# danping/CoSLAM

Hardware: AMD Instinct MI355X
Metric: frames/sec for track+local-BA loop, 8 cams 640x480 x 2000 feats (one frame = all 8 cameras) (higher is better)
Workload: dtype f32 (KLT, f16 pyramid storage) + f64 (pose, BA)

## Files before the change

coslam_amd/csrc/klt_detect.hip:

```cpp
#include "klt_front_dev.h"

#pragma clang fp contract(off)


namespace {

__device__ __forceinline__ void suppress_at(float* corner, int W, int H, float s, float t) {
    if (!(s >= 0.0f && t >= 0.0f)) return;
    float fx = floorf(s * (float)W), fy = floorf(t * (float)H);
    if (fx >= (float)W || fy >= (float)H) return;
    corner[(size_t)(int)fy * W + (int)fx] = -1e30f;
}

__global__ void k_suppress_list(float* corner, int W, int H, int n, const float* __restrict__ list3) {
    int k = blockIdx.x * blockDim.x + threadIdx.x;
    if (k < n) suppress_at(corner, W, H, list3[3 * k], list3[3 * k + 1]);
}

__global__ void k_post_track(const float* __restrict__ feat, int N, cs_klt_feature* __restrict__ dest, int* ctr,
                             float* corner, int W, int H, int doSuppress) {
    int i = blockIdx.x * blockDim.x + threadIdx.x;
    if (i >= N) return;
    float X = feat[3 * i], Y = feat[3 * i + 1], gain = feat[3 * i + 2];
    if (X >= 0) {
        dest[i].status = 0;
        dest[i].pos[0] = X;
        dest[i].pos[1] = Y;
        dest[i].gain = gain;
        dest[i].fed = -1;
        if (doSuppress) suppress_at(corner, W, H, X, Y);
    } else {
        dest[i].status = -1;
        dest[i].fed = -1;
    }
}

__global__ void k_clear_dest(cs_klt_feature* dest, int N) {
    int i = blockIdx.x * blockDim.x + threadIdx.x;
    if (i < N) {
        dest[i].status = -1;
        dest[i].fed = -1;
    }
}

constexpr int NTW = 64, NTH = 16;

__device__ __forceinline__ unsigned part1by1(unsigned v) {
    v &= 0xffffu;
    v = (v | (v << 8)) & 0x00ff00ffu;
    v = (v | (v << 4)) & 0x0f0f0f0fu;
    v = (v | (v << 2)) & 0x33333333u;
    v = (v | (v << 1)) & 0x55555555u;
    return v;
}

struct CsNonmaxArgs {
    const float* in;
    int W, H, d;
    float* out;
    CsCand* cand;
    int maxCand;
    int* ctr;
};

__device__ __forceinline__ void nonmax_body(const CsNonmaxArgs& Z, int bx, int by, int tid, float* smem) {
    const float* __restrict__ in = Z.in;
    float* __restrict__ out = Z.out;
    CsCand* __restrict__ cand = Z.cand;
    int* ctr = Z.ctr;
    const int W = Z.W, H = Z.H, d = Z.d, maxCand = Z.maxCand;
    const int RW = NTW + 2 * d, RH = NTH + 2 * d;
    float* raw = smem;
    float* rowres = smem + RH * RW;
    const int x0 = bx * NTW, y0 = by * NTH;
    for (int base = tid; base < RH * RW; base += 8 * 256) {
        float tv[8];
#pragma unroll
        for (int u = 0; u < 8; ++u) {
            const int i = base + 256 * u;
            const int ly = i / RW, lx = i - ly * RW;
            const int gx = cs_clampi(x0 + lx - d, 0, W - 1), gy = cs_clampi(y0 + ly - d, 0, H - 1);
            tv[u] = in[(size_t)gy * W + gx];
        }
#pragma unroll
        for (int u = 0; u < 8; ++u) {
            const int i = base + 256 * u;
            if (i < RH * RW) raw[i] = tv[u];
        }
    }
    __syncthreads();
    for (int i = tid; i < RH * NTW; i += 256) {
        int ly = i / NTW, lx = i - ly * NTW;
        const float* r = raw + ly * RW + lx + d;
        float m = r[0];
        for (int k = -d; k < 0; ++k) {
            float cn = fabsf(r[k]);
            m = (cn >= fabsf(m)) ? (-cn) : m;
        }
        for (int k = 1; k <= d; ++k) {
            float cn = fabsf(r[k]);
            m = (cn >= fabsf(m)) ? (-cn) : m;
        }
        rowres[i] = m;
    }
    __syncthreads();
    const int lx = tid & (NTW - 1), x = x0 + lx;
    for (int ly = tid / NTW; ly < NTH; ly += 256 / NTW) {
        int y = y0 + ly;
        if (x >= W || y >= H) continue;
        const float* r = rowres + (ly + d) * NTW + lx;
        float m = r[0];
        for (int k = -d; k < 0; ++k) {
            float cn = fabsf(r[k * NTW]);
            m = (cn >= fabsf(m)) ? (-cn) : m;
        }
        for (int k = 1; k <= d; ++k) {
            float cn = fabsf(r[k * NTW]);
            m = (cn >= fabsf(m)) ? (-cn) : m;
        }
        out[(size_t)y * W + x] = m;
        if (m > 0.0f) {
            int slot = atomicAdd(&ctr[0], 1);
            if (slot < maxCand) {
                CsCand cd;
                cd.key = part1by1((unsigned)x) | (part1by1((unsigned)y) << 1);
                cd.x = ((float)x + 0.5f) / (float)W;
                cd.y = ((float)y + 0.5f) / (float)H;
                cd.c = m;
                cand[slot] = cd;
            }
        }
    }
}

struct CsNonmaxBatch {
    int W, H, d, maxCand;
    CsNonmaxCam cam[CS_MAX_CAMS];
};
__device__ __forceinline__ CsNonmaxArgs nonmax_args(const CsNonmaxBatch& B, int c) {
    CsNonmaxArgs Z = {B.cam[c].in, B.W, B.H, B.d, B.cam[c].out, B.cam[c].cand, B.maxCand, B.cam[c].ctr};
    return Z;
}

__global__ __launch_bounds__(256) void k_nonmax_compact(CsNonmaxBatch B) {
    extern __shared__ __attribute__((aligned(16))) float smem[];
    nonmax_body(nonmax_args(B, blockIdx.z), blockIdx.x, blockIdx.y, threadIdx.x, smem);
}

struct CsSelectArgs {
    const CsCand* cand;
    int maxCand, cap, maxKeepFixed;
    int* rankM;
    CsCand* sel;
};

__device__ __forceinline__ void select_fill_body(const CsSelectArgs& Q, const CsFillArgs& A) {
    __shared__ float cs[1024];
    __shared__ unsigned ks[1024];
    __shared__ int rs[1024];
    __shared__ int part[1024];
    const int tid = threadIdx.x;
    const int N = A.N;
    __shared__ int nTrackedSh;
    {
        int c = 0;
        if (A.mode == 2)
            for (int i = tid; i < N; i += 1024) c += (A.dest[i].status >= 0) ? 1 : 0;
        part[tid] = c;
        __syncthreads();
        for (int s = 512; s > 0; s >>= 1) {
            if (tid < s) part[tid] += part[tid + s];
            __syncthreads();
        }
        if (tid == 0) nTrackedSh = part[0];
        __syncthreads();
    }
    const int nTracked = nTrackedSh;
    const int n = min(A.ctr[0], Q.maxCand);
    const int nK = min(n, Q.cap);
    int maxKeep = (Q.maxKeepFixed >= 0) ? Q.maxKeepFixed : (N - nTracked);
    if (maxKeep < 0) maxKeep = 0;
    const int nSel = min(nK, maxKeep);
    for (int i0 = 0; i0 < n; i0 += 1024) {
        const int i = i0 + tid;
        const unsigned ki = (i < n) ? Q.cand[i].key : 0u;
        int r = 0;
        for (int base = 0; base < n; base += 1024) {
            const int j = base + tid;
            ks[tid] = (j < n) ? Q.cand[j].key : 0xffffffffu;
            __syncthreads();
            const int m = min(1024, n - base);
            for (int q = 0; q < m; ++q) r += (ks[q] < ki) ? 1 : 0;
            __syncthreads();
        }
        if (i < n) Q.rankM[i] = r;
    }
    __syncthreads();
    for (int i0 = 0; i0 < n; i0 += 1024) {
        const int i = i0 + tid;
        CsCand me;
        me.key = 0;
        me.x = me.y = me.c = 0;
        int myRank = 0x7fffffff;
        if (i < n) {
            me = Q.cand[i];
            myRank = Q.rankM[i];
        }
        if (nK <= maxKeep) {
            if (i < n && myRank < nK) Q.sel[myRank] = me;
            continue;
        }
        int r = 0;
        for (int base = 0; base < n; base += 1024) {
            const int j = base + tid;
            const bool ok = (j < n);
            cs[tid] = ok ? Q.cand[j].c : 0.0f;
            ks[tid] = ok ? Q.cand[j].key : 0u;
            rs[tid] = ok ? Q.rankM[j] : 0x7fffffff;
            __syncthreads();
            const int m = min(1024, n - base);
            for (int q = 0; q < m; ++q) {
                const bool in = rs[q] < nK;
                const bool before = (cs[q] > me.c) || (cs[q] == me.c && ks[q] < me.key);
                r += (in && before) ? 1 : 0;
            }
            __syncthreads();
        }
        if (i < n && myRank < nK && r < maxKeep) Q.sel[r] = me;
    }
    __syncthreads();
    const int chunk = (N + 1023) / 1024;
    const int lo = min(tid * chunk, N), hi = min(lo + chunk, N);
    int nDead = 0;
    for (int i = lo; i < hi; ++i) nDead += (A.mode == 2) ? (A.dest[i].status < 0 ? 1 : 0) : 1;
    part[tid] = nDead;
    __syncthreads();
    for (int s = 1; s < 1024; s <<= 1) {
        int v = (tid >= s) ? part[tid - s] : 0;
        __syncthreads();
        part[tid] += v;
        __syncthreads();
    }
    int r = part[tid] - nDead;
    for (int i = lo; i < hi; ++i) {
        bool dead = (A.mode == 2) ? (A.dest[i].status < 0) : true;
        float lx, ly, lz;
        if (dead) {
            if (r < nSel) {
                CsCand c = Q.sel[r];
                cs_klt_feature f;
                f.status = 1;
                f.pos[0] = c.x;
                f.pos[1] = c.y;
                f.gain = (A.mode == 2) ? c.c : (A.withGain ? 1.0f : c.c);
                f.fed = -1;
                A.dest[i] = f;
                lx = c.x;
                ly = c.y;
                lz = (A.mode == 2 || A.withGain) ? 1.0f : c.c;
            } else if (A.mode == 1 && r < nSel + A.nPresentGiven) {
                int q = r - nSel;
                cs_klt_feature f;
                f.status = 1;
                f.pos[0] = A.present3[3 * q];
                f.pos[1] = A.present3[3 * q + 1];
                f.gain = A.withGain ? 1.0f : 0.0f;
                f.fed = q;
                A.dest[i] = f;
                lx = f.pos[0];
                ly = f.pos[1];
                lz = f.gain;
            } else {
                A.dest[i].status = -1;
                if (A.mode != 1) A.dest[i].fed = -1;
                lx = ly = -1.0f;
                lz = (A.mode == 2 || A.withGain) ? 1.0f : -1.0f;
            }
            ++r;
        } else {
            lx = A.dest[i].pos[0];
            ly = A.dest[i].pos[1];
            lz = 1.0f;
        }
        A.list_a[3 * i] = lx;
        A.list_a[3 * i + 1] = ly;
        A.list_a[3 * i + 2] = lz;
        if (A.list_b) {
            A.list_b[3 * i] = lx;
            A.list_b[3 * i + 1] = ly;
            A.list_b[3 * i + 2] = lz;
        }
    }
    if (tid == 0) {
        int nPres = (A.mode == 2) ? nTracked : (A.mode == 1 ? min(A.nPresentGiven, max(N - nSel, 0)) : 0);
        A.ctr[1] = nTracked;
        A.ctr[2] = nSel;
        A.counts[0] = nSel + nPres;
        A.counts[1] = (A.mode == 2) ? nTracked : 0;
        A.counts[2] = A.ctr[0];
        A.counts[3] = nSel;
        A.ctr[0] = 0;
    }
    if (A.tagWord && tid == 0) *A.tagWord += 1u;
}

struct CsSelectBatch {
    int maxCand, cap;
    CsSelectCam cam[CS_MAX_CAMS];
};
__device__ __forceinline__ CsSelectArgs select_args(const CsSelectBatch& B, int c) {
    CsSelectArgs Q = {B.cam[c].cand, B.maxCand, B.cap, B.cam[c].maxKeepFixed, B.cam[c].rankM, B.cam[c].sel};
    return Q;
}

__global__ __launch_bounds__(1024) void k_select_fill(CsSelectBatch B) {
    select_fill_body(select_args(B, blockIdx.x), B.cam[blockIdx.x].fill);
}

struct CsLevel0Batch {
    int W, H;
    float minCornerness, lox, loy, hix, hiy;
    int nbx, nby;
    CsFrontCam cam[CS_MAX_CAMS];
};

__global__ __launch_bounds__(256) void k_tail_nonmax_level0(CsNonmaxBatch Z, int nax, int nA, CsLevel0Batch Y) {
    extern __shared__ __attribute__((aligned(16))) float smem[];
    const int b = blockIdx.x, c = blockIdx.y;
    if (b < nA) {
        nonmax_body(nonmax_args(Z, c), b % nax, b / nax, threadIdx.x, smem);
    } else {
        const int q = b - nA;
        const CsFrontCam& F = Y.cam[c];
        cs_level0_body<true>(F.img, Y.W, Y.H, F.pyr, F.corner, Y.minCornerness, Y.lox, Y.loy, Y.hix, Y.hiy, nullptr, q % Y.nbx,
                             q / Y.nbx, Y.nbx, Y.nby, threadIdx.x, *(CsLevel0Lds<true>*)smem);
    }
}

struct CsTailPyr {
    cs_texel* pyr[CS_MAX_CAMS];
};
__global__ __launch_bounds__(1024) void k_tail_select_down(CsSelectBatch B, CsTailPyr P, CsDownFused F, int ntx, int nty) {
    extern __shared__ __attribute__((aligned(16))) unsigned char down_smem[];
    const int c = blockIdx.y;
    if (blockIdx.x == 0) {
        select_fill_body(select_args(B, c), B.cam[c].fill);
        return;
    }
    if (threadIdx.x >= 256) return;
    const int t = blockIdx.x - 1;
    cs_down_body(P.pyr[c], F, t % ntx, t / ntx, threadIdx.x, (cs_texel*)down_smem, true);
}

__global__ __launch_bounds__(1024) void k_counts_track(const cs_klt_feature* __restrict__ dest, int N, int* counts, int* ctr,
                                                       unsigned* tagWord) {
    __shared__ int part[1024];
    const int tid = threadIdx.x;
    int c = 0;
    for (int i = tid; i < N; i += 1024) c += (dest[i].status >= 0) ? 1 : 0;
    part[tid] = c;
    __syncthreads();
    for (int s = 512; s > 0; s >>= 1) {
        if (tid < s) part[tid] += part[tid + s];
        __syncthreads();
    }
    if (tid == 0) {
        counts[0] = part[0];
        counts[1] = part[0];
        counts[2] = 0;
        counts[3] = 0;
        if (ctr) ctr[0] = 0;
    }
    if (tagWord && tid == 0) *tagWord += 1u;
}

}

int cs_launch_suppress_list(float* corner, int W, int H, int n, const float* d_list3, hipStream_t stream) {
    if (n <= 0) return CS_OK;
    hipLaunchKernelGGL(k_suppress_list, dim3((n + 255) / 256), dim3(256), 0, stream, corner, W, H, n, d_list3);
    CS_CHECK_LAUNCH();
    return CS_OK;
}

int cs_launch_post_track(const float* feat, int N, cs_klt_feature* dest, int* ctr, float* corner, int W, int H,
                         int doSuppress, hipStream_t stream) {
    hipLaunchKernelGGL(k_post_track, dim3((N + 255) / 256), dim3(256), 0, stream, feat, N, dest, ctr, corner, W, H,
                       doSuppress);
    CS_CHECK_LAUNCH();
    return CS_OK;
}

int cs_launch_clear_dest(cs_klt_feature* dest, int N, hipStream_t stream) {
    hipLaunchKernelGGL(k_clear_dest, dim3((N + 255) / 256), dim3(256), 0, stream, dest, N);
    CS_CHECK_LAUNCH();
    return CS_OK;
}

size_t cs_nonmax_lds_bytes(int d) { return sizeof(float) * ((size_t)(NTH + 2 * d) * (NTW + 2 * d) + (size_t)(NTH + 2 * d) * NTW); }

static int fill_nonmax_batch(CsNonmaxBatch& B, const CsNonmaxCam* cams, int n, int W, int H, int d, int maxCand) {
    if (n < 1 || n > CS_MAX_CAMS) {
        cs_set_error("detector: %d cameras (1..%d)", n, CS_MAX_CAMS);
        return CS_ERR_INVALID;
    }
    memset(&B, 0, sizeof(B));
    B.W = W;
    B.H = H;
    B.d = d;
    B.maxCand = maxCand;
    for (int c = 0; c < n; ++c) B.cam[c] = cams[c];
    return CS_OK;
}
static void fill_select_batch(CsSelectBatch& B, const CsSelectCam* cams, int n, int maxCand, int cap) {
    memset(&B, 0, sizeof(B));
    B.maxCand = maxCand;
    B.cap = cap;
    for (int c = 0; c < n; ++c) B.cam[c] = cams[c];
}

int cs_launch_nonmax_compact(const CsNonmaxCam* cams, int n, int W, int H, int d, int maxCand, hipStream_t stream) {
    size_t lds = cs_nonmax_lds_bytes(d);
    if (lds > 160 * 1024) {
        cs_set_error("minDistance %d needs %zu B of LDS (> 160 KiB)", d, lds);
        return CS_ERR_INVALID;
    }
    CsNonmaxBatch B;
    int rc = fill_nonmax_batch(B, cams, n, W, H, d, maxCand);
    if (rc) return rc;
    dim3 grid((W + NTW - 1) / NTW, (H + NTH - 1) / NTH, n);
    hipLaunchKernelGGL(k_nonmax_compact, grid, dim3(256), lds, stream, B);
    CS_CHECK_LAUNCH();
    return CS_OK;
}

int cs_nonmax_prepare(int d) {
    size_t lds = cs_nonmax_lds_bytes(d);
    if (lds > 64 * 1024) {
        hipError_t e = hipFuncSetAttribute((const void*)k_nonmax_compact, hipFuncAttributeMaxDynamicSharedMemorySize,
                                           (int)lds);
        if (e != hipSuccess) {
            cs_set_error("hipFuncSetAttribute(maxDynamicShared=%zu) failed: %s", lds, hipGetErrorString(e));
            return CS_ERR_HIP;
        }
    }
    return CS_OK;
}

int cs_launch_select_fill(const CsSelectCam* cams, int n, int maxCand, int cap, hipStream_t stream) {
    if (n < 1 || n > CS_MAX_CAMS) {
        cs_set_error("selection: %d cameras (1..%d)", n, CS_MAX_CAMS);
        return CS_ERR_INVALID;
    }
    CsSelectBatch B;
    fill_select_batch(B, cams, n, maxCand, cap);
    hipLaunchKernelGGL(k_select_fill, dim3(n), dim3(1024), 0, stream, B);
    CS_CHECK_LAUNCH();
    return CS_OK;
}

int cs_launch_counts_track(const cs_klt_feature* dest, int N, int* counts, int* ctr, unsigned* tagWord, hipStream_t stream) {
    hipLaunchKernelGGL(k_counts_track, dim3(1), dim3(1024), 0, stream, dest, N, counts, ctr, tagWord);
    CS_CHECK_LAUNCH();
    return CS_OK;
}

int cs_launch_tail_with_next_front(const CsNonmaxCam* nm, const CsSelectCam* sel, const CsFrontCam* next, int n, int W, int H,
                                   int d, int maxCand, int cap, const CsPyrLayout& lay, int tap_mode, float minCornerness,
                                   float margin, hipStream_t stream) {
    size_t ldsA = cs_nonmax_lds_bytes(d);
    if (ldsA < sizeof(CsLevel0Lds<true>)) ldsA = sizeof(CsLevel0Lds<true>);
    if (ldsA > 64 * 1024) {
        cs_set_error("fused detector tail: minDistance %d needs %zu B of LDS", d, ldsA);
        return CS_ERR_INVALID;
    }
    CsNonmaxBatch Z;
    int rc = fill_nonmax_batch(Z, nm, n, W, H, d, maxCand);
    if (rc) return rc;
    const int nax = (W + NTW - 1) / NTW, nay = (H + NTH - 1) / NTH;
    CsLevel0Batch Y;
    memset(&Y, 0, sizeof(Y));
    Y.W = W;
    Y.H = H;
    Y.minCornerness = minCornerness;
    Y.lox = margin / (float)W;
    Y.loy = margin / (float)H;
    Y.hix = 1.0f - margin / (float)W;
    Y.hiy = 1.0f - margin / (float)H;
    Y.nbx = (W + FTW - 1) / FTW;
    Y.nby = (H + FTH - 1) / FTH;
    CsTailPyr P;
    memset(&P, 0, sizeof(P));
    for (int c = 0; c < n; ++c) {
        Y.cam[c] = next[c];
        P.pyr[c] = next[c].pyr;
    }
    hipLaunchKernelGGL(k_tail_nonmax_level0, dim3(nax * nay + Y.nbx * Y.nby, n), dim3(256), ldsA, stream, Z, nax, nax * nay, Y);
    CsSelectBatch B;
    fill_select_batch(B, sel, n, maxCand, cap);
    if (lay.L >= 2) {
        CsDownFused F;
        int ntx, nty;
        size_t lds;
        rc = cs_down_fused_plan(lay, tap_mode, &F, &ntx, &nty, &lds);
        if (rc) return rc;
        hipLaunchKernelGGL(k_tail_select_down, dim3(1 + ntx * nty, n), dim3(1024), lds, stream, B, P, F, ntx, nty);
        rc = cs_launch_pyr_down_tail(P.pyr, n, lay, tap_mode, F.NL + 1, stream);
        if (rc) return rc;
    } else {
        hipLaunchKernelGGL(k_select_fill, dim3(n), dim3(1024), 0, stream, B);
    }
    CS_CHECK_LAUNCH();
    return CS_OK;
}
```

include/coslam_hip.h:

```cpp
#ifndef COSLAM_HIP_H
#define COSLAM_HIP_H

#include <stddef.h>
#include <stdint.h>

#ifdef __cplusplus
extern "C" {
#endif

#define CS_OK 0
#define CS_ERR_INVALID (-1)
#define CS_ERR_NO_DEVICE (-2)
#define CS_ERR_HIP (-3)
#define CS_ERR_ALLOC (-4)
#define CS_ERR_NUMERIC (-5)

int cs_version(void);
const char* cs_last_error(void);
int cs_debug_set(const char* key, int value);
int cs_device_count(void);


typedef struct cs_klt_feature {
    int status;
    float pos[2];
    float gain;
    int fed;
} cs_klt_feature;

typedef struct cs_klt_config {
    int nIterations, nLevels, levelSkip, windowWidth;
    float trackBorderMargin, convergenceThreshold, SSD_Threshold;
    int trackWithGain;
    int minDistance;
    float minCornerness, detectBorderMargin;
} cs_klt_config;

void cs_klt_config_default(cs_klt_config* cfg);

typedef struct cs_klt cs_klt;

cs_klt* cs_klt_create(const cs_klt_config* cfg, int device, int tap_mode);
void cs_klt_destroy(cs_klt* k);

int cs_klt_allocate(cs_klt* k, int width, int height, int nLevels, int featuresWidth, int featuresHeight,
                    int pointListWidth, int pointListHeight);
int cs_klt_deallocate(cs_klt* k);

int cs_klt_set_border_margin(cs_klt* k, float margin);
int cs_klt_set_convergence_threshold(cs_klt* k, float thr);
int cs_klt_set_ssd_threshold(cs_klt* k, float thr);

int cs_klt_detect(cs_klt* k, const uint8_t* image, int* nDetectedFeatures, cs_klt_feature* dest);
int cs_klt_detect_present(cs_klt* k, const uint8_t* image, int* nDetectedFeatures, cs_klt_feature* dest, int nPresent,
                          const float* present);
int cs_klt_redetect(cs_klt* k, const uint8_t* image, int* nNewFeatures, cs_klt_feature* dest);
int cs_klt_track(cs_klt* k, const uint8_t* image, int* nPresentFeatures, cs_klt_feature* dest);
int cs_klt_redetect_async_h(cs_klt* k, const unsigned char* image);
int cs_klt_fetch(cs_klt* k, int* nNew, cs_klt_feature* dest);
int cs_klt_feed(cs_klt* k, int npts, const float* featPts, int* trackIds, int* nFed);
int cs_klt_feed_dev(cs_klt* k, int npts, const float* d_featPts, int* d_trackIds, int* d_nFed);
int cs_klt_advance(cs_klt* k);

int cs_klt_set_stream(cs_klt* k, void* hip_stream);
int cs_klt_detect_dev(cs_klt* k, const void* d_image, void* d_dest, void* d_counts);
int cs_klt_redetect_dev(cs_klt* k, const void* d_image, void* d_dest, void* d_counts);
int cs_klt_track_dev(cs_klt* k, const void* d_image, void* d_dest, void* d_counts);
int cs_klt_prefetch_dev(cs_klt* k, const void* d_image_next);
int cs_klt_synchronize(cs_klt* k);
int cs_klt_enable_graphs(cs_klt* k, int on);
int cs_klt_set_fused(cs_klt* k, int on);
int cs_klt_set_cu_count(cs_klt* k, int n_cus);
int cs_klt_set_xcd_placement(cs_klt* k, int on);
int cs_klt_set_concurrent_handles(cs_klt* k, int n);
void* cs_stream_create_cu_range(int device, int first_cu, int n_cus);
void* cs_stream_create_cu_interleaved(int device, int period, int take, int complement);
int cs_stream_destroy(void* stream);
int cs_klt_debug_probe(cs_klt* k, int on, unsigned long long* host_out8);
int cs_klt_set_profiling(cs_klt* k, int on);
int cs_klt_get_profile(cs_klt* k, double* tracker_us_total, int* n_frames, int* launches_per_frame);

typedef struct cs_klt_group cs_klt_group;
cs_klt_group* cs_klt_group_create(cs_klt* const* handles, int n);
void cs_klt_group_destroy(cs_klt_group* g);
int cs_klt_group_size(const cs_klt_group* g);
int cs_klt_group_set_stream(cs_klt_group* g, void* hip_stream);
int cs_klt_group_detect_dev(cs_klt_group* g, const void* const* d_images, void* const* d_dests, void* const* d_counts);
int cs_klt_group_redetect_dev(cs_klt_group* g, const void* const* d_images, void* const* d_dests, void* const* d_counts);
int cs_klt_group_track_dev(cs_klt_group* g, const void* const* d_images, void* const* d_dests, void* const* d_counts);
int cs_klt_group_prefetch_dev(cs_klt_group* g, const void* const* d_images_next);
int cs_klt_group_stage_h(cs_klt_group* g, const unsigned char* const* h_images, int* slot);
int cs_klt_group_staged(cs_klt_group* g, int slot, const void** d_images);
void* cs_pinned_alloc(size_t bytes);
void cs_pinned_free(void* p);
int cs_klt_group_advance(cs_klt_group* g);
int cs_klt_group_synchronize(cs_klt_group* g);

size_t cs_klt_pyramid_texels(const cs_klt* k);
int cs_klt_pyramid_level_offset(const cs_klt* k, int level, int64_t* off_texels, int* w, int* h);
int cs_klt_read_pyramid(cs_klt* k, int which, uint16_t* host_out);
int cs_klt_read_cornerness(cs_klt* k, float* host_out);
int cs_klt_read_features(cs_klt* k, float* host_out3);
int cs_klt_build_pyramid(cs_klt* k, const uint8_t* image);


typedef struct cs_pose_option {
    int maxIterLM, maxIterRW;
    double epsErrorChangeLM, epsParamChangeLM, epsErrorChangeRW;
    int verboseLM, verboseRW;
    double lambda0, lambda;
    double err0, err, errRW;
    int retTypeLM, npts, nIterLM, nIterRW;
} cs_pose_option;

void cs_pose_option_default(cs_pose_option* opt);

int cs_pose_intracam(const double K[9], const double R0[9], const double t0[3], int npts, const double* prevErrs,
                     const double* Ms, const double* ms, double tau, double R_opt[9], double t_opt[3],
                     cs_pose_option* opt, int device);

int cs_pose_intracam_batch_dev(int device, void* hip_stream, int nProb, int ptsStride, const double* K,
                               const double* R0, const double* t0, const int* npts, const double* prevErrs,
                               const double* Ms, const double* ms, double tau, double* R_opt, double* t_opt,
                               cs_pose_option* opt, int* ok);

typedef struct cs_handback_cam {
    const cs_klt_feature* dest;
    const double* K;
    const double* kud;
    const double* mapPts;
    const unsigned char* isStatic;
    int* slot2map;
    int* trackSpan;
    double* xy;
    int* state;
    int* selBlk;
    double* Ms;
    double* ms;
    int* sel;
    int* npts;
    cs_pose_option* opt;
    int* pointFeat;
    int pointFeatStride, nPointFeat;
} cs_handback_cam;
int cs_klt_handback_dev(int device, void* hip_stream, int nCams, const cs_handback_cam* cams, int N, int W, int H,
                        int nColBlk, int nRowBlk, int ptsStride, int frame );

typedef struct cs_klt_hostview cs_klt_hostview;
cs_klt_hostview* cs_klt_hostview_create(int device, cs_klt* const* handles, int nCams, int W, int H, int N, const double* K,
                                        const double* kud, int depth );
void cs_klt_hostview_destroy(cs_klt_hostview* v);
unsigned char* cs_klt_hostview_image(cs_klt_hostview* v, int cam);
int cs_klt_hostview_frame(cs_klt_hostview* v, const unsigned char* const* h_images, int frame, int first);
int cs_klt_hostview_fetch(cs_klt_hostview* v, int frame, const int** state, const double** xy);
int cs_klt_hostview_oldest(const cs_klt_hostview* v);
int cs_klt_hostview_newest(const cs_klt_hostview* v);
int cs_klt_hostview_synchronize(cs_klt_hostview* v);

typedef struct cs_register_cam {
    const double* K;
    const double* R;
    const double* t;
    const double* xy;
    const int* state;
    const int* slot2map;
    const unsigned char* isDynamic;
    const unsigned char* isStatic;
} cs_register_cam;
typedef struct cs_register_pass {
    int P;
    double sigmaSearch, maxDist, sigmaMerge;
    const double* M;
    const double* cov;
    const int* pointFeat;
    int* slot;
    double* m;
    double* var;
    double* dist;
    int* flags;
    const unsigned char* mapFlags;
    double maxDistDynamic;
    const int* list;
} cs_register_pass;
int cs_register_list_current_dev(int device, void* hip_stream, int nCams, int nMap, const int* d_mapCount, const int* d_pointFeat,
                                 const unsigned char* d_mapFlags, int* d_list, int* d_listCount, int* d_slotTable);
int cs_register_list_current_cap_dev(int device, void* hip_stream, int nCams, int nMap, const int* d_mapCount, const int* d_pointFeat,
                                     const unsigned char* d_mapFlags, int* d_list, int* d_listCount, int* d_slotTable, int listCap,
                                     int* d_overflow);
int cs_register_search_passes_dev(int device, void* hip_stream, int nCams, const cs_register_cam* cams, int N, int W, int H,
                                  int nPass , const cs_register_pass* passes );
int cs_register_search_passes_range_dev(int device, void* hip_stream, int nCams, int cam0, int nCamsRun, const cs_register_cam* cams,
                                        int N, int W, int H, int nPass, const cs_register_pass* passes);
int cs_register_search_dev(int device, void* hip_stream, int nCams, const cs_register_cam* cams, int N, int W, int H, int P,
                           const double* d_M, const double* d_cov, const int* d_pointFeat, double sigmaSearch, double maxDist,
                           double sigmaMerge, int* d_slot, double* d_m, double* d_var, double* d_dist, int* d_flags);
int cs_register_search(int device, int nCams, const cs_register_cam* cams, int N, int W, int H, int P, const double* M,
                       const double* cov, const int* pointFeat, double sigmaSearch, double maxDist, double sigmaMerge, int* slot,
                       double* m, double* var, double* dist, int* flags);

size_t cs_register_decide_scratch_bytes(int nCams, int N, int P);
int cs_register_decide_static_dev(int device, void* hip_stream, int nCams, int N, int P, int mapBase, const int* d_slot, const int* d_flags,
                                  const unsigned char* d_mergeable, const unsigned char* d_mapFlags, int* d_pointFeat,
                                  int* const* d_slot2map , unsigned char* d_attached,
                                  unsigned char* d_regged, void* d_scratch, int nSweeps, int* d_counts);
int cs_register_decide_static_cam_dev(int device, void* hip_stream, int nCams, int N, int P, int mapBase, const int* d_slot, const int* d_flags,
                                      const unsigned char* d_mergeable, const unsigned char* d_mapFlags, int* d_pointFeat,
                                      int* const* d_slot2map, unsigned char* d_attached, unsigned char* d_regged, void* d_scratch, int nSweeps,
                                      int* d_counts, int onlyCam);
int cs_register_decide_kinds_dev(int device, void* hip_stream, int nCams, int N, int P, int mapBase, const int* d_slot, const int* d_flags,
                                 const unsigned char* d_mergeable, const unsigned char* d_mapFlags, int* d_pointFeat, int* const* d_slot2map,
                                 unsigned char* d_attached, unsigned char* d_regged, void* d_scratch, int nSweeps, int* d_counts, int onlyCam,
                                 int kinds);

int cs_register_revisit_list_dev(int device, void* hip_stream, int nCams, int P, int cap, int firstRound, const int* d_pointFeat,
                                 const unsigned char* d_attached, unsigned char* d_regIn, int keepIn, unsigned char* d_regOutClear ,
                                 int* d_visitLoop, int* d_nextLoop, int* d_list, int* d_counts);
int cs_register_revisit_decide_dev(int device, void* hip_stream, int nCams, int N, int P, int cap, int mapBase, int kinds, const int* d_list,
                                   const int* d_nextLoop, int* d_visitLoop, const int* d_slot, const int* d_flags, const unsigned char* d_mergeable,
                                   const unsigned char* d_mapFlags, int* d_pointFeat, int* const* d_slot2map, unsigned char* d_attached,
                                   unsigned char* d_regOut, void* d_decideScratch, const int* d_curList, const int* d_curCount, int curCap,
                                   int* d_counts, const int* d_listCount );

int cs_register_decide_kinds_rounds_dev(int device, void* hip_stream, int nCams, int N, int P, int mapBase, const int* d_slot, const int* d_flags,
                                        const unsigned char* d_mergeable, const unsigned char* d_mapFlags, int* d_pointFeat, int* const* d_slot2map,
                                        unsigned char* d_attached, unsigned char* d_regged, void* d_scratch, int nSweeps, int* d_counts, int onlyCam,
                                        int kinds, int* d_rvLists, int rvCap, int nRounds, int* d_rvCounts, int* d_visitLoop, int* d_nextLoop);
int cs_register_revisit_decide_next_dev(int device, void* hip_stream, int nCams, int N, int P, int cap, int mapBase, int kinds, const int* d_list,
                                        int* d_nextLoop, int* d_visitLoop, const int* d_slot, const int* d_flags, const unsigned char* d_mergeable,
                                        const unsigned char* d_mapFlags, int* d_pointFeat, int* const* d_slot2map, unsigned char* d_attached,
                                        unsigned char* d_regOut, void* d_decideScratch, const int* d_curList, const int* d_curCount, int curCap,
                                        int* d_counts, const int* d_listCount, int* d_nextList, int* d_nextCount, int* d_overflow);

int cs_register_candidates_pack_dev(int device, void* hip_stream, int P, int nCams, int cam0, int nOwn, const int* d_slot, const int* d_flags,
                                    const unsigned char* d_mergeable, int* d_send);
int cs_register_candidates_unpack_dev(int device, void* hip_stream, int P, int nCams, int nOwn, int skipRank, const int* d_recv, int* d_slot,
                                      int* d_flags, unsigned char* d_mergeable);
int cs_register_candidates_pack_list_dev(int device, void* hip_stream, int cap, int nCams, int cam0, int nOwn, const int* d_list, const int* d_slot,
                                         const int* d_flags, const unsigned char* d_mergeable, int* d_send);
int cs_register_candidates_unpack_list_dev(int device, void* hip_stream, int cap, int nCams, int nOwn, int skipRank, const int* d_list,
                                           const int* d_recv, int* d_slot, int* d_flags, unsigned char* d_mergeable);

#define CS_MAP_DYNAMIC 1
#define CS_MAP_FALSE 2
#define CS_MAP_UNCERTAIN 4
typedef struct cs_poseupdate_cam {
    const double* K;
    const double* iK;
    const double* xy;
    const int* state;
    const int* slot2map;
    const int* trackSpan;
    double* reprojErr;
    unsigned char* isStatic;
} cs_poseupdate_cam;
typedef struct cs_track_history cs_track_history;
cs_track_history* cs_track_history_create(int device, int nCams, int N, int histLen );
cs_track_history* cs_track_history_create_ex(int device, int nCams, int N, int histLen, int storeLen);
void cs_track_history_destroy(cs_track_history* h);
int cs_track_history_frames(const cs_track_history* h);
int cs_pose_update3d_dev(int device, void* hip_stream, int nCams, int cam0, int nCamsRun, const cs_poseupdate_cam* cams, int N,
                         const int* d_pointFeat, int nMap, const double* d_R, const double* d_t, double* d_mapPts, double* d_mapCov,
                         unsigned char* d_mapFlags, int largeErr, double pixelErrVar, int* d_numNodes, int* d_numOut);
int cs_detect_dynamic_dev(cs_track_history* h, void* hip_stream, int cam0, int nCamsRun, const cs_poseupdate_cam* cams,
                          const double* d_R, const double* d_t, int nMap, const unsigned char* d_mapFlags, int frame, int maxLen,
                          int minLen, int minOutNum, double maxEpiErr, int* d_numDyn);
int cs_pose_update_frame_dev(cs_track_history* h, void* hip_stream, const cs_poseupdate_cam* cams, const int* d_pointFeat, int nMap,
                             const double* d_R, const double* d_t, double* d_mapPts, double* d_mapCov, unsigned char* d_mapFlags,
                             int largeErr, double pixelErrVar, int frame, int maxLen, int minLen, int minOutNum, double maxEpiErr,
                             int* d_numNodes, int* d_numOut, int* d_numDyn);

int cs_register_mergability_dev(const cs_track_history* h, void* hip_stream, const cs_poseupdate_cam* cams, int P, const double* d_M,
                                const double* d_cov, const int* d_slot, double pixelErrVar, unsigned char* d_mergeable);

int cs_register_mergability_range_dev(const cs_track_history* h, void* hip_stream, int cam0, int nCamsRun, const cs_poseupdate_cam* cams,
                                      int P, const double* d_M, const double* d_cov, const int* d_slot, double pixelErrVar,
                                      unsigned char* d_mergeable);
size_t cs_register_mergability_cache_bytes(int P, int nCams);
int cs_register_mergability_running_dev(const cs_track_history* h, void* hip_stream, int cam0, int nCamsRun, const cs_poseupdate_cam* cams,
                                        int P, const double* d_M, const double* d_cov, const int* d_slot, double pixelErrVar, double tolPix,
                                        void* d_cache, unsigned char* d_mergeable, int* d_counts);
int cs_register_mergability_running_list_dev(const cs_track_history* h, void* hip_stream, int cam0, int nCamsRun, const cs_poseupdate_cam* cams,
                                             int P, const int* d_list, int nList, const double* d_M, const double* d_cov, const int* d_slot,
                                             const int* d_flags, double pixelErrVar, double tolPix, void* d_cache, unsigned char* d_mergeable,
                                             int* d_counts);

int cs_track_history_set_poses_dev(cs_track_history* h, void* hip_stream, int n, const int* d_cam, const int* d_frame, const double* d_R,
                                   const double* d_t);
int cs_track_history_get_span_dev(const cs_track_history* h, void* hip_stream, int firstFrame, int nFrames, double* d_R, double* d_t);
int cs_track_history_set_span_dev(cs_track_history* h, void* hip_stream, int firstFrame, int nFrames, const double* d_R, const double* d_t);
int cs_track_history_newest_frame(const cs_track_history* h);
int cs_track_history_cams(const cs_track_history* h);
int cs_update_new_poses_points_dev(const cs_track_history* h, void* hip_stream, const cs_poseupdate_cam* cams, const int* d_pointFeat,
                                   int nMap, const int* d_lastFrame, const unsigned char* d_isCurrent, int firstKeyFrame,
                                   double* d_mapPts, double* d_mapCov, const unsigned char* d_mapFlags, double pixelErrVar,
                                   int* d_counts);
int cs_refine_map_points_dev(const cs_track_history* h, void* hip_stream, const cs_poseupdate_cam* cams, const int* d_pointFeat, int nMap,
                             const unsigned char* d_select, double* d_mapPts, double* d_mapCov, double pixelErrVar, int* d_count);

size_t cs_newpts_intracam_scratch_bytes(int nCams, int N);
int cs_newpts_intracam_dev(const cs_track_history* h, void* hip_stream, const cs_poseupdate_cam* cams, const int* d_ready, int readyMin,
                           int minTrackLen, int maxWalk, double maxEpiErr, double pixelErrVar, double* d_mapPts, double* d_mapCov,
                           unsigned char* d_mapFlags, unsigned char* d_newPt, int* d_firstFrame, int* d_pointFeat, int mapCap, int* d_mapCount,
                           void* d_scratch, int* d_counts);

typedef struct {
    const int* state;
    const int* slot2map;
    const double* R;
    const double* t;
    int* keyFrame;
    int* keyMapped;
    double* selfR;
    double* selfT;
} cs_keyframe_cam;
int cs_keyframe_ready_dev(int device, void* hip_stream, int nCams, int N, const cs_keyframe_cam* cams, int nMap, const double* d_mapPts,
                          const unsigned char* d_mapFlags, const int* d_firstFrame, int curFrame, double ratio, double minViewAngleDeg,
                          double minTranslation, int addKeyFrame, int* d_ready, int* d_mapped, double* d_center, int* d_stats);

int cs_keyframe_snapshot_dev(int device, void* hip_stream, int nCams, int N, const double* d_xy, const int* d_state, const int* d_slot2map,
                             const double* d_R, const double* d_t, const int* d_word, double* d_xyOut, int* d_stateOut, int* d_slot2mapOut,
                             double* d_ROut, double* d_tOut, int* h_word);

typedef struct { int slot, frame, first, seg; } cs_feat_ref;
typedef struct { int slot, last, first, next; } cs_feat_seg;
int cs_feat_ref_advance_dev(cs_track_history* h, void* hip_stream, const cs_poseupdate_cam* cams, int nMap, const int* d_pointFeat,
                            int curFrame, cs_feat_ref* d_featRef, unsigned char* d_refStatic, int* d_counts);
int cs_feat_ref_advance_list_dev(cs_track_history* h, void* hip_stream, const cs_poseupdate_cam* cams, int nMap, const int* d_pointFeat,
                                 int curFrame, cs_feat_ref* d_featRef, unsigned char* d_refStatic, int* d_counts, const int* d_list, int nList);
int cs_feat_ref_advance_refine_dev(cs_track_history* h, void* hip_stream, const cs_poseupdate_cam* cams, int nMap, const int* d_pointFeat,
                                   int curFrame, cs_feat_ref* d_featRef, unsigned char* d_refStatic, int* d_counts, const int* d_list, int nList,
                                   int advanceAll, unsigned char* d_select, int clearSelect, double* d_mapPts, double* d_mapCov,
                                   double pixelErrVar);
int cs_track_history_segments(const cs_track_history* h, cs_feat_seg** d_pool, int* cap, int** d_count);
int cs_track_history_segment_counts(const cs_track_history* h, int* counts);
int cs_track_history_load_segments(cs_track_history* h, const cs_feat_seg* segs, int n);
int cs_track_history_download_segments(const cs_track_history* h, cs_feat_seg* segs, int n);
int cs_update_new_poses_points_ref_dev(const cs_track_history* h, void* hip_stream, const cs_poseupdate_cam* cams, const cs_feat_ref* d_featRef,
                                       const unsigned char* d_refStatic, int nMap, const int* d_lastFrame, const unsigned char* d_isCurrent,
                                       int firstKeyFrame, double* d_mapPts, double* d_mapCov, const unsigned char* d_mapFlags, double pixelErrVar,
                                       int* d_counts);
int cs_refine_map_points_ref_dev(const cs_track_history* h, void* hip_stream, const cs_poseupdate_cam* cams, const cs_feat_ref* d_featRef,
                                 int nMap, const unsigned char* d_select, double* d_mapPts, double* d_mapCov, double pixelErrVar, int* d_count);

int cs_track_history_set_classify_refs(cs_track_history* h, cs_feat_ref* d_featRef, unsigned char* d_refStatic);

int cs_track_history_set_merge_refs(cs_track_history* h, cs_feat_ref* d_featRef, unsigned char* d_refStatic);

int cs_check_unify_dev(const cs_track_history* h, void* hip_stream, const cs_poseupdate_cam* cams, int nPairs, const int* d_pf1,
                       const int* d_pf2, const double* d_M1, const double* d_M2, double pixelErrVar, unsigned char* d_ok, double* d_M,
                       double* d_cov);
int cs_check_unify_ref_dev(const cs_track_history* h, void* hip_stream, const cs_poseupdate_cam* cams, int nPairs, const cs_feat_ref* d_ref1,
                           const cs_feat_ref* d_ref2, const double* d_M1, const double* d_M2, double pixelErrVar, unsigned char* d_ok, double* d_M,
                           double* d_cov);
int cs_register_decide_merge_dev(const cs_track_history* h, void* hip_stream, const cs_poseupdate_cam* cams, int P, int mapBase, const int* d_slot,
                                 const int* d_flags, const unsigned char* d_mergeable, unsigned char* d_mapFlags, int* d_pointFeat, double* d_mapPts,
                                 double* d_mapCov, double pixelErrVar, unsigned char* d_attached, unsigned char* d_regged, void* d_scratch,
                                 int* d_counts, int onlyCam);
size_t cs_register_decide_merge_scratch_bytes(int P, int nList, int nCams);
int cs_register_decide_merge_list_dev(const cs_track_history* h, void* hip_stream, const cs_poseupdate_cam* cams, int P, int mapBase,
                                      const int* d_list, int nList, const int* d_slot, const int* d_flags, const unsigned char* d_mergeable,
                                      unsigned char* d_mapFlags, int* d_pointFeat, double* d_mapPts, double* d_mapCov, double pixelErrVar,
                                      unsigned char* d_attached, unsigned char* d_regged, void* d_scratch, int* d_counts, int onlyCam);


int cs_map_points_classify_dev(const cs_track_history* h, void* hip_stream, const cs_poseupdate_cam* cams, int* d_pointFeat, int nMap,
                               const int* d_featFrame, const int* d_featFirst, int curFrame, double* d_mapPts, double* d_mapCov,
                               unsigned char* d_mapFlags, unsigned char* d_newPt, int* d_staticFrameNum, const int* d_firstFrame,
                               double pixelVar, int* d_counts);
int cs_pose_update_classify_frame_dev(cs_track_history* h, void* hip_stream, const cs_poseupdate_cam* cams, int* d_pointFeat, int nMap,
                                      const double* d_R, const double* d_t, double* d_mapPts, double* d_mapCov, unsigned char* d_mapFlags,
                                      int largeErr, double pixelErrVar, int frame, int maxLen, int minLen, int minOutNum, double maxEpiErr,
                                      int* d_numNodes, int* d_numOut, int* d_numDyn, const int* d_featFrame, const int* d_featFirst,
                                      unsigned char* d_newPt, int* d_staticFrameNum, const int* d_firstFrame, double pixelVarClassify,
                                      int* d_clsCounts);

typedef struct cs_posegraph cs_posegraph;
int cs_posegraph_create(int device, int nGraphs, const int* nodePtr, const int* edgePtr, const unsigned char* fixed,
                        const int* id1, const int* id2, cs_posegraph** out);
void cs_posegraph_destroy(cs_posegraph* g);
int cs_posegraph_counts(const cs_posegraph* g, int* nNodes, int* nEdges, int* nComponents, int* maxHalfBandwidth);
int cs_posegraph_relax_dev(cs_posegraph* g, void* hip_stream, const double* d_nodeR, const double* d_nodeT,
// ... 246 lines not shown
```

Measured before the change: 1087.

## Replace quadratic rank-counting selection with LDS bitonic sort in select_fill

The candidate ranking step in select_fill used an O(n^2) all-pairs comparison to rank candidates by key, then again by cornerness. It now packs key/index into 64-bit words and bitonic-sorts them in LDS, with a second sort on inverted cornerness when only a subset is kept. The O(n^2) path is kept as a fallback for n beyond the sort capacity. The dead-slot prefix scan is also replaced with a wave-shuffle scan, and a standalone select_fill entry point is added. The cost is a larger LDS footprint (up to 128KB in k_select_fill, and at least 16KB in the fused kernel), which can lower occupancy. The 16-bit index packing also assumes candidate counts below 65536.

```diff
diff --git a/coslam_amd/csrc/klt_detect.hip b/coslam_amd/csrc/klt_detect.hip
--- a/coslam_amd/csrc/klt_detect.hip
+++ b/coslam_amd/csrc/klt_detect.hip
@@ -154,100 +154,162 @@
     CsCand* sel;
 };
 
-__device__ __forceinline__ void select_fill_body(const CsSelectArgs& Q, const CsFillArgs& A) {
-    __shared__ float cs[1024];
-    __shared__ unsigned ks[1024];
-    __shared__ int rs[1024];
-    __shared__ int part[1024];
+__device__ __forceinline__ void bitonic_sort_lds(unsigned long long* buf, int P, int tid) {
+    for (int k = 2; k <= P; k <<= 1) {
+        for (int j = k >> 1; j > 0; j >>= 1) {
+            for (int t = tid; t < (P >> 1); t += 1024) {
+                const int i = 2 * t - (t & (j - 1)), l = i + j;
+                const unsigned long long a = buf[i], b = buf[l];
+                if ((a > b) == ((i & k) == 0)) {
+                    buf[i] = b;
+                    buf[l] = a;
+                }
+            }
+            const int jNext = (j > 1) ? (j >> 1) : k;
+            if (j >= 128 || (jNext >= 128 && (k << 1) <= P) || (j == 1 && k == P)) {
+                __syncthreads();
+            } else {
+                __builtin_amdgcn_fence(__ATOMIC_RELEASE, "wavefront");
+                __builtin_amdgcn_wave_barrier();
+                __builtin_amdgcn_fence(__ATOMIC_ACQUIRE, "wavefront");
+            }
+        }
+    }
+}
+
+__device__ __forceinline__ int pow2_at_least(int n) {
+    int P = 2;
+    while (P < n) P <<= 1;
+    return P;
+}
+
+__device__ __forceinline__ void select_fill_body(const CsSelectArgs& Q, const CsFillArgs& A, unsigned long long* sortBuf,
+                                                 int sortCap) {
     const int tid = threadIdx.x;
     const int N = A.N;
-    __shared__ int nTrackedSh;
+    const int n = min(A.ctr[0], Q.maxCand);
+    __shared__ int waveDead[16];
+    const int chunk = (N + 1023) / 1024;
+    const int lo = min(tid * chunk, N), hi = min(lo + chunk, N);
+    int nDead = 0;
+    for (int i = lo; i < hi; ++i) nDead += (A.mode == 2) ? (A.dest[i].status < 0 ? 1 : 0) : 1;
+    int deadBefore, nTracked;
     {
-        int c = 0;
-        if (A.mode == 2)
-            for (int i = tid; i < N; i += 1024) c += (A.dest[i].status >= 0) ? 1 : 0;
-        part[tid] = c;
+        const int lane = tid & 63, wave = tid >> 6;
+        int v = nDead;
+        for (int o = 1; o < 64; o <<= 1) {
+            const int y = __shfl_up(v, o, 64);
+            if (lane >= o) v += y;
+        }
+        if (lane == 63) waveDead[wave] = v;
         __syncthreads();
-        for (int s = 512; s > 0; s >>= 1) {
-            if (tid < s) part[tid] += part[tid + s];
-            __syncthreads();
-        }
-        if (tid == 0) nTrackedSh = part[0];
-        __syncthreads();
-    }
-    const int nTracked = nTrackedSh;
-    const int n = min(A.ctr[0], Q.maxCand);
+        int before = 0, total = 0;
+        for (int w = 0; w < 16; ++w) {
+            const int x = waveDead[w];
+            before += (w < wave) ? x : 0;
+            total += x;
+        }
+        deadBefore = before + v - nDead;
+        nTracked = (A.mode == 2) ? N - total : 0;
+    }
     const int nK = min(n, Q.cap);
     int maxKeep = (Q.maxKeepFixed >= 0) ? Q.maxKeepFixed : (N - nTracked);
     if (maxKeep < 0) maxKeep = 0;
     const int nSel = min(nK, maxKeep);
-    for (int i0 = 0; i0 < n; i0 += 1024) {
-        const int i = i0 + tid;
-        const unsigned ki = (i < n) ? Q.cand[i].key : 0u;
-        int r = 0;
-        for (int base = 0; base < n; base += 1024) {
-            const int j = base + tid;
-            ks[tid] = (j < n) ? Q.cand[j].key : 0xffffffffu;
+    const bool sorted = (n <= sortCap);
+    if (sorted) {
+        const int P = pow2_at_least(n);
+        for (int i = tid; i < P; i += 1024)
+            sortBuf[i] = (i < n) ? (((unsigned long long)Q.cand[i].key << 32) | (unsigned)i) : ~0ull;
+        __syncthreads();
+        bitonic_sort_lds(sortBuf, P, tid);
+        const bool all = (nK <= maxKeep);
+        for (int r = tid; r < n; r += 1024) {
+            const int i = (int)(unsigned)sortBuf[r];
+            Q.rankM[i] = r;
+            if (all && r < nK) Q.sel[r] = Q.cand[i];
+            if (all) sortBuf[r] &= 0xffffu;
+        }
+        if (!all) {
+            const int P2 = pow2_at_least(nK);
+            for (int r = tid; r < P2; r += 1024) {
+                unsigned long long w = ~0ull;
+                if (r < nK) {
+                    const unsigned i = (unsigned)sortBuf[r];
+                    const unsigned cb = __float_as_uint(Q.cand[i].c);
+                    w = ((unsigned long long)(~cb & 0x7fffffffu) << 32) | ((unsigned)r << 16) | i;
+                }
+                sortBuf[r] = w;
+            }
             __syncthreads();
-            const int m = min(1024, n - base);
-            for (int q = 0; q < m; ++q) r += (ks[q] < ki) ? 1 : 0;
-            __syncthreads();
-        }
-        if (i < n) Q.rankM[i] = r;
-    }
-    __syncthreads();
-    for (int i0 = 0; i0 < n; i0 += 1024) {
-        const int i = i0 + tid;
-        CsCand me;
-        me.key = 0;
-        me.x = me.y = me.c = 0;
-        int myRank = 0x7fffffff;
-        if (i < n) {
-            me = Q.cand[i];
-            myRank = Q.rankM[i];
-        }
-        if (nK <= maxKeep) {
-            if (i < n && myRank < nK) Q.sel[myRank] = me;
-            continue;
-        }
-        int r = 0;
-        for (int base = 0; base < n; base += 1024) {
-            const int j = base + tid;
-            const bool ok = (j < n);
-            cs[tid] = ok ? Q.cand[j].c : 0.0f;
-            ks[tid] = ok ? Q.cand[j].key : 0u;
-            rs[tid] = ok ? Q.rankM[j] : 0x7fffffff;
-            __syncthreads();
-            const int m = min(1024, n - base);
-            for (int q = 0; q < m; ++q) {
-                const bool in = rs[q] < nK;
-                const bool before = (cs[q] > me.c) || (cs[q] == me.c && ks[q] < me.key);
-                r += (in && before) ? 1 : 0;
-            }
-            __syncthreads();
-        }
-        if (i < n && myRank < nK && r < maxKeep) Q.sel[r] = me;
-    }
-    __syncthreads();
-    const int chunk = (N + 1023) / 1024;
-    const int lo = min(tid * chunk, N), hi = min(lo + chunk, N);
-    int nDead = 0;
-    for (int i = lo; i < hi; ++i) nDead += (A.mode == 2) ? (A.dest[i].status < 0 ? 1 : 0) : 1;
-    part[tid] = nDead;
-    __syncthreads();
-    for (int s = 1; s < 1024; s <<= 1) {
-        int v = (tid >= s) ? part[tid - s] : 0;
+            bitonic_sort_lds(sortBuf, P2, tid);
+            for (int r = tid; r < nSel; r += 1024) {
+                const unsigned i = (unsigned)sortBuf[r] & 0xffffu;
+                Q.sel[r] = Q.cand[i];
+                sortBuf[r] = i;
+            }
+        }
         __syncthreads();
-        part[tid] += v;
+    } else {
+        float* cs = (float*)sortBuf;
+        unsigned* ks = (unsigned*)(cs + 1024);
+        int* rs = (int*)(ks + 1024);
+        for (int i0 = 0; i0 < n; i0 += 1024) {
+            const int i = i0 + tid;
+            const unsigned ki = (i < n) ? Q.cand[i].key : 0u;
+            int r = 0;
+            for (int base = 0; base < n; base += 1024) {
+                const int j = base + tid;
+                ks[tid] = (j < n) ? Q.cand[j].key : 0xffffffffu;
+                __syncthreads();
+                const int m = min(1024, n - base);
+                for (int q = 0; q < m; ++q) r += (ks[q] < ki) ? 1 : 0;
+                __syncthreads();
+            }
+            if (i < n) Q.rankM[i] = r;
+        }
         __syncthreads();
-    }
-    int r = part[tid] - nDead;
+        for (int i0 = 0; i0 < n; i0 += 1024) {
+            const int i = i0 + tid;
+            CsCand me;
+            me.key = 0;
+            me.x = me.y = me.c = 0;
+            int myRank = 0x7fffffff;
+            if (i < n) {
+                me = Q.cand[i];
+                myRank = Q.rankM[i];
+            }
+            if (nK <= maxKeep) {
+                if (i < n && myRank < nK) Q.sel[myRank] = me;
+                continue;
+            }
+            int r = 0;
+            for (int base = 0; base < n; base += 1024) {
+                const int j = base + tid;
+                const bool ok = (j < n);
+                cs[tid] = ok ? Q.cand[j].c : 0.0f;
+                ks[tid] = ok ? Q.cand[j].key : 0u;
+                rs[tid] = ok ? Q.rankM[j] : 0x7fffffff;
+                __syncthreads();
+                const int m = min(1024, n - base);
+                for (int q = 0; q < m; ++q) {
+                    const bool in = rs[q] < nK;
+                    const bool before = (cs[q] > me.c) || (cs[q] == me.c && ks[q] < me.key);
+                    r += (in && before) ? 1 : 0;
+                }
+                __syncthreads();
+            }
+            if (i < n && myRank < nK && r < maxKeep) Q.sel[r] = me;
+        }
+        __syncthreads();
+    }
+    int r = deadBefore;
     for (int i = lo; i < hi; ++i) {
         bool dead = (A.mode == 2) ? (A.dest[i].status < 0) : true;
         float lx, ly, lz;
         if (dead) {
             if (r < nSel) {
-                CsCand c = Q.sel[r];
+                const CsCand c = sorted ? Q.cand[(unsigned)sortBuf[r]] : Q.sel[r];
                 cs_klt_feature f;
                 f.status = 1;
                 f.pos[0] = c.x;
@@ -313,8 +375,11 @@
     return Q;
 }
 
+constexpr int SELECT_SORT_CAP = 16384;
+constexpr size_t SELECT_FUSED_LDS = 2048 * sizeof(unsigned long long);
 __global__ __launch_bounds__(1024) void k_select_fill(CsSelectBatch B) {
-    select_fill_body(select_args(B, blockIdx.x), B.cam[blockIdx.x].fill);
+    __shared__ unsigned long long sortBuf[SELECT_SORT_CAP];
+    select_fill_body(select_args(B, blockIdx.x), B.cam[blockIdx.x].fill, sortBuf, SELECT_SORT_CAP);
 }
 
 struct CsLevel0Batch {
@@ -340,11 +405,12 @@
 struct CsTailPyr {
     cs_texel* pyr[CS_MAX_CAMS];
 };
-__global__ __launch_bounds__(1024) void k_tail_select_down(CsSelectBatch B, CsTailPyr P, CsDownFused F, int ntx, int nty) {
+__global__ __launch_bounds__(1024) void k_tail_select_down(CsSelectBatch B, CsTailPyr P, CsDownFused F, int ntx, int nty,
+                                                          int sortCap) {
     extern __shared__ __attribute__((aligned(16))) unsigned char down_smem[];
     const int c = blockIdx.y;
     if (blockIdx.x == 0) {
-        select_fill_body(select_args(B, c), B.cam[c].fill);
+        select_fill_body(select_args(B, c), B.cam[c].fill, (unsigned long long*)down_smem, sortCap);
         return;
     }
     if (threadIdx.x >= 256) return;
@@ -504,7 +570,10 @@
         size_t lds;
         rc = cs_down_fused_plan(lay, tap_mode, &F, &ntx, &nty, &lds);
         if (rc) return rc;
-        hipLaunchKernelGGL(k_tail_select_down, dim3(1 + ntx * nty, n), dim3(1024), lds, stream, B, P, F, ntx, nty);
+        if (lds < SELECT_FUSED_LDS) lds = SELECT_FUSED_LDS;
+        int sortCap = 2048;
+        while ((size_t)sortCap * 2 * sizeof(unsigned long long) <= lds) sortCap *= 2;
+        hipLaunchKernelGGL(k_tail_select_down, dim3(1 + ntx * nty, n), dim3(1024), lds, stream, B, P, F, ntx, nty, sortCap);
         rc = cs_launch_pyr_down_tail(P.pyr, n, lay, tap_mode, F.NL + 1, stream);
         if (rc) return rc;
     } else {
@@ -513,3 +582,30 @@
     CS_CHECK_LAUNCH();
     return CS_OK;
 }
+
+extern "C" int cs_klt_select_fill_dev(const void* d_cand, int maxCand, int cap, int maxKeepFixed, int mode, int N, int withGain,
+                                      int nPresentGiven, const float* d_present3, void* d_dest, int* d_ctr, int* d_rankM,
+                                      void* d_sel, float* d_list, int* d_counts, void* hip_stream) {
+    if (!d_cand || !d_dest || !d_ctr || !d_rankM || !d_sel || !d_list || !d_counts || maxCand < 1 || N < 1 || mode < 0 ||
+        mode > 2 || (mode == 1 && nPresentGiven > 0 && !d_present3)) {
+        cs_set_error("cs_klt_select_fill_dev: bad arguments");
+        return CS_ERR_INVALID;
+    }
+    CsSelectCam c;
+    memset(&c, 0, sizeof(c));
+    c.cand = (const CsCand*)d_cand;
+    c.rankM = d_rankM;
+    c.sel = (CsCand*)d_sel;
+    c.maxKeepFixed = maxKeepFixed;
+    c.fill.mode = mode;
+    c.fill.N = N;
+    c.fill.withGain = withGain;
+    c.fill.nPresentGiven = nPresentGiven;
+    c.fill.present3 = d_present3;
+    c.fill.sel = c.sel;
+    c.fill.ctr = d_ctr;
+    c.fill.dest = (cs_klt_feature*)d_dest;
+    c.fill.list_a = d_list;
+    c.fill.counts = d_counts;
+    return cs_launch_select_fill(&c, 1, maxCand, cap, (hipStream_t)hip_stream);
+}
diff --git a/include/coslam_hip.h b/include/coslam_hip.h
--- a/include/coslam_hip.h
+++ b/include/coslam_hip.h
@@ -77,6 +77,9 @@
 void* cs_stream_create_cu_interleaved(int device, int period, int take, int complement);
 int cs_stream_destroy(void* stream);
 int cs_klt_debug_probe(cs_klt* k, int on, unsigned long long* host_out8);
+int cs_klt_select_fill_dev(const void* d_cand, int maxCand, int cap, int maxKeepFixed, int mode, int N, int withGain,
+                           int nPresentGiven, const float* d_present3, void* d_dest, int* d_ctr, int* d_rankM, void* d_sel,
+                           float* d_list, int* d_counts, void* hip_stream);
 int cs_klt_set_profiling(cs_klt* k, int on);
 int cs_klt_get_profile(cs_klt* k, double* tracker_us_total, int* n_frames, int* launches_per_frame);
 
```

New measurement: 1100, median of 6. About the same (+1.2%).
